# arkCyber/whisper-rust

Measured on AMD Instinct MI355X. Metric: real-time factor (audio-sec/wall-sec), greedy, 30 s synthetic chunks, higher is better.
Workload: dtype f16 operands / f32 accumulate; 1 GPU; ggml-small-shaped synthetic F16 model, greedy best_of=1 temperature_inc=0, 1 x 30 s 16 kHz f32 chunk per GPU, PCM resident in HBM; flash_attn=False, parallelism=chunk-dp1

## Files before the change

### whisper-rust_amd/csrc/wa_mega.h

```cpp
#pragma once
#include "wa_kernels.h"

struct wa_mega_layer {
    const float * ln1_w, * ln1_b; const wa_f16 * qkv_w; const float * qkv_b, * qkv_s;
    const wa_f16 * out_w;  const float * out_b;
    const float * ln2_w, * ln2_b; const wa_f16 * cq_w;  const float * cq_b;
    const wa_f16 * co_w;   const float * co_b;
    const float * ln3_w, * ln3_b; const wa_f16 * fc1_w; const float * fc1_b;
    const wa_f16 * fc2_w;  const float * fc2_b;
    const float * qkv_d, * out_d, * cq_d, * co_d, * fc1_d, * fc2_d;
};

struct wa_mega_args {
    const wa_mega_layer * layers; int n_layer, d, n_head, n_vocab; float eps;
    double rn_d;
    const wa_f16 * te; const float * pe; const float * lnf_w, * lnf_b; const wa_f16 * gelu;
    const float * te_d; int quant;
    wa_f16 * kv_k, * kv_v; unsigned long long kv_layer_stride;
    const wa_f16 * cross_k, * cross_v; unsigned long long cross_layer_stride;
    int cross_tpad, T;
    unsigned long long * granules; int edge_stride;
    unsigned long long * cross_gr;
    float * logits;
    unsigned * status;
// ... 30 lines not shown
        if (b < nG) { role = 0; idx = b; } else if (b < nG + H) { role = 1; idx = b - nG; } else { role = 2; idx = b - nG - H; }
        return;
    }
    if (b >= top) {
        const int t = b - top, r = t & 7, k = t >> 3, q = k >> 2, w = k & 3, h = r + 8 * q;
        if (h < H) { role = 2; idx = 4 * h + w; return; }
        const int f = (r - R) + (8 - R) * w;
        if (f < H) { role = 1; idx = f; } else { role = 0; idx = (top - s_low) + (f - H); }
        return;
    }
    if (b >= top - s_low) { role = 1; idx = F + (b - (top - s_low)); } else { role = 0; idx = b; }
}

bool   wa_launch_decode_mega(hipStream_t s, const wa_mega_args & a, int n_wg);
size_t wa_mega_lds_bytes();
```

### whisper-rust_amd/csrc/wa_mega.hip

```cpp
#include "wa_device.h"
#include "wa_mega.h"

typedef unsigned long long u64;
#define GAS __attribute__((address_space(1)))
typedef GAS u64 gu64;
typedef GAS unsigned gu32;
typedef const GAS wa_f16 * gch;
typedef const GAS float * gcf;
typedef _Float16 half4v __attribute__((ext_vector_type(4)));
typedef unsigned u32x2 __attribute__((ext_vector_type(2)));
typedef unsigned u32x4 __attribute__((ext_vector_type(4)));

typedef const __attribute__((address_space(4))) wa_mega_args * mg_kargs;
__device__ __forceinline__ mg_kargs mg_uniform(mg_kargs p) {
    const unsigned long long v = (unsigned long long) p;
    const unsigned lo = __builtin_amdgcn_readfirstlane((unsigned) v), hi = __builtin_amdgcn_readfirstlane((unsigned) (v >> 32));
    return (mg_kargs) (((unsigned long long) hi << 32) | lo);
}

#define MG_THREADS 512
#define MG_NW (MG_THREADS / 64)
#define MG_NP3 4
#define MG_SPIN_LIMIT 20000u
#ifndef MG_DEFER
// ... 75 lines not shown
        if ((spins & 127u) == 127u) {
            const unsigned st = __builtin_amdgcn_readfirstlane(__hip_atomic_load(c.status, __ATOMIC_RELAXED, __HIP_MEMORY_SCOPE_AGENT));
            if (st != 0u) { c.dead = true; return spins; }
            if (spins >= MG_SPIN_LIMIT) {
                if (lane == 0) __hip_atomic_store(c.status, code, __ATOMIC_RELAXED, __HIP_MEMORY_SCOPE_AGENT);
                c.dead = true;
                return spins;
            }
        }
        __builtin_amdgcn_s_sleep(1);
    }
}

#define MG_WGTRACE_LAYER 4
#define MG_NQ 6
#define MG_EX_P1 (MG_DEFER ? 0x06u : 0x20u)
#define MG_EX_P4 (MG_DEFER ? 0x06u : 0x08u)
#define MG_EX_P7 (BIGP ? 0x18u : MG_DEFER && !QB ? 0x10u : 0x08u)
#define MG_EX_AO 0x06u
#define MG_EX_AO2 0x10u
#define MG_EX_HF (MG_DEFER ? 0x08u : 0x06u)
#define MG_EX_HFQ 0x18u
#define MG_EX_FINAL 0x20u
__device__ __forceinline__ int mg_slot(int wave, unsigned ex) {
    if ((ex >> wave) & 1u) return -1;
    const int sl = __builtin_popcount(~ex & ((1u << wave) - 1u) & 0xffu);
    return sl < MG_NQ ? sl : -1;
}
__device__ __forceinline__ int mg_seg(int n) { return ((n + MG_NQ - 1) / MG_NQ + 31) & ~31; }
__device__ __forceinline__ int mg_ln_seg(int d) { return mg_seg(d); }
template <int NP3>
__device__ __forceinline__ void mg_ln_params(float (&gw)[NP3], float (&gb)[NP3], const float * lw, const float * lb, int d, int q, int lane) {
    const int seg = mg_ln_seg(d), i0 = q * seg, i1 = min(d, i0 + seg);
#pragma unroll
    for (int k = 0; k < NP3; ++k) {
        const int i = i0 + lane + 64 * k;
// ... 92 lines not shown
            else if (i < i1) xin[i] = f2h(y);
        }
        if (tslot >= 0) mg_trace(A, lane == 0, tslot + 2, mg_now());
    }
    mg_barrier();
}

template <int NPL>
__device__ __forceinline__ void mg_gather_h2(mg_ctl & c, gu64 * edge, int i0, int i1, int lane, unsigned * dst32, unsigned code, mg_kargs A = nullptr,
                                             int tslot = -1) {
    unsigned v[NPL];
    const unsigned sp = mg_sweep<NPL>(edge, [&](int k) { const int i = i0 + lane + 64 * k; return i < i1 ? i : -1; }, c, lane, v, code);
    if (tslot >= 0) { mg_trace(A, lane == 0, tslot, mg_now()); mg_trace(A, lane == 0, tslot + 1, sp); }
#pragma unroll
    for (int k = 0; k < NPL; ++k) { const int i = i0 + lane + 64 * k; if (i < i1) dst32[i] = v[k]; }
}

template <int NPL>
__device__ __forceinline__ void mg_gather_q8(mg_ctl & c, gu64 * edge, int i0, int i1, int lane, wa_f16 * xin, int nb, unsigned code, mg_kargs A = nullptr,
                                             int tslot = -1) {
    unsigned v[NPL];
    const unsigned sp = mg_sweep<NPL>(edge, [&](int k) { const int i = i0 + lane + 64 * k; return i < i1 ? i : -1; }, c, lane, v, code);
    if (tslot >= 0) { mg_trace(A, lane == 0, tslot, mg_now()); mg_trace(A, lane == 0, tslot + 1, sp); }
    const int ln = mq_fresh(lane);
    unsigned * q32 = (unsigned *) mq_xq(xin) + ((ln & 31) >> 2) * mq_ld(nb) + (i0 >> 5) + (ln >> 5);
    float * dsc = mq_xd(xin) + (i0 >> 5) + (ln >> 5);
#pragma unroll
    for (int k = 0; k < NPL; ++k) mq_put(__uint_as_float(v[k]), i0 + ln + 64 * k < i1, q32 + 2 * k, dsc + 2 * k, ln);
}

// ... 410 lines not shown
                                sl = __uint_as_float(rb[lane * 8 + 4]); ml = s2.v; }
            mg_best_wave(t2); mg_best_wave(s2);
            float sg = ml > -INFINITY ? sl * __expf(ml - s2.v) : 0.0f;
            sg = wave_sum(sg);
            if (lane == 0) {
                GAS unsigned * ro = (GAS unsigned *) A->rec_out + (size_t) wg * 8;
                ro[0] = __float_as_uint(t2.v); ro[1] = (unsigned) t2.i; ro[2] = __float_as_uint(s2.v); ro[3] = (unsigned) s2.i; ro[4] = __float_as_uint(sg);
            }
        }
    }
    mg_trace(A, blockIdx.x == 0 && wave == 0 && lane == 0, (A->n_layer * 8) * 8 + 3, mg_now());
    if (A->dbg) { mg_trace(A, blockIdx.x == 0 && wave == 0 && lane == 0, 3022, (unsigned) clock64()); mg_trace(A, blockIdx.x == 0 && wave == 0 && lane == 0, 3023, mg_now()); }
    if (blockIdx.x == 0 && wave == 0 && lane == 0) ((GAS unsigned *) A->logits)[A->n_vocab + 2] = c.seq;
}

template <int NP3, int NS, bool Q = false>
__device__ __forceinline__ void mg_role_gemv(mg_kargs A_, int idx_) {
    extern __shared__ __attribute__((aligned(16))) unsigned char smem[];
    const mg_kargs A = mg_uniform(A_);
    int lane = threadIdx.x & 63;
#define MG_FRESH() do { lane = mq_fresh(lane); } while (0)
    const int wave = __builtin_amdgcn_readfirstlane(threadIdx.x >> 6);
    const int wg = __builtin_amdgcn_readfirstlane(idx_), nG = (int) gridDim.x - 5 * A->n_head;
    mg_ctl c; c.status = (gu32 *) A->status; c.seq = A->seq; c.dead = false;
    mg_chaos_start(c.seq);
    mg_trace(A, wg == 0 && wave == 0 && (threadIdx.x & 63) == 0, (A->n_layer * 8) * 8 + 6, mg_now());
    if (A->dbg) { mg_trace(A, wg == 0 && wave == 0 && (threadIdx.x & 63) == 0, 3020, (unsigned) clock64()); mg_trace(A, wg == 0 && wave == 0 && (threadIdx.x & 63) == 0, 3021, mg_now()); }
    unsigned pf[96];
    bool have_pf = false;
    constexpr bool BIG = NP3 == MG_NP3;
    constexpr bool QB = Q && !BIG && MG_DEFER;
    constexpr bool BIGP = BIG && MG_DEFER;
    float    * fc1x   = (float *) (smem + WA_MEGA_MAX_D * 4 + 7 * WA_MEGA_MAX_D);
    unsigned * fc1cnt = (unsigned *) (smem + WA_MEGA_MAX_D * 4 + 7 * WA_MEGA_MAX_D + 128);

    float  * xf  = (float *) smem;
    wa_f16 * xin = (wa_f16 *) (smem + WA_MEGA_MAX_D * 4);
    wa_f16 * xinB = (wa_f16 *) (smem + MG_XINB_OFF);
    const int d = A->d, L = A->n_layer, d4 = 4 * d;
    const int r_qkv = mg_rpw(3 * d, nG), r_d = mg_rpw(d, nG), r_ff = mg_rpw(d4, nG);
    const int row_qkv = wg * r_qkv, row_d = wg * r_d, row_ff = wg * r_ff;
    const int g_qkv = (r_qkv + 7) >> 3, g_ff = (r_ff + 7) >> 3, g_d8 = (r_d + 7) >> 3, g_d16 = (r_d + 3) >> 2;
    const __attribute__((address_space(4))) wa_mega_layer * Ly = (const __attribute__((address_space(4))) wa_mega_layer *) A->layers;
    const unsigned seq = c.seq;
    const int kv_head = A->kv_head;

    double * lnred = (double *) (smem + MG_LNRED_OFF);
    wa_f16 * gelu_l = (wa_f16 *) (smem + MG_GELU_OFF);
    float gw[NP3], gb[NP3];
    int * pk = (int *) (smem + MG_PICK_OFF);
    mg_ln_params<NP3>(gw, gb, Ly[0].ln1_w, Ly[0].ln1_b, d, mg_slot(wave, MG_EX_P1), lane);
    if (wave == 0) mg_pick(A, lane, pk);
    if (QB && wave == 0 && lane == 0) *fc1cnt = 0u;
    mg_task t; t.valid = false; t.row = 0; t.wrow = nullptr; t.bias = 0.f; t.scale = 1.f;
    if (wave == 1 || wave == 2) t = mg_mk8<Q, NS>(pf, Ly[0].qkv_w, Ly[0].qkv_d, Ly[0].qkv_b, Ly[0].qkv_s, 3 * d, d, row_qkv, r_qkv, wave - 1, lane);
    else if (wave == 3)         t = mg_mk8<Q, NS>(pf, Ly[0].out_w, Ly[0].out_d, Ly[0].out_b, nullptr, d, d, row_d, r_d, 0, lane);
    else if (wave == 4)         t = mg_mk8<Q, NS>(pf, Ly[0].cq_w, Ly[0].cq_d, Ly[0].cq_b, nullptr, d, d, row_d, r_d, 0, lane);
    else if (wave == 5)         t = mg_mk16<Q, 4 * NS>(pf, Ly[0].fc2_w, Ly[0].fc2_d, Ly[0].fc2_b, d, d4, row_d, r_d, 0, lane);
    else if (wave >= 6 && !(BIGP && L > 0)) mg_prefetch_logits<NS, Q>(A, pf, have_pf, lane, wave);
    mg_barrier();
    mg_trace(A, wg == 0 && wave == 0 && lane == 0, (A->n_layer * 8) * 8 + 7, mg_now());
    if (wave >= 3 && wave <= 5) {
        const GAS u32x4 * src = (const GAS u32x4 *) A->gelu;
        for (int j = wave - 3; j < 128; j += 3)
            __builtin_amdgcn_global_load_lds((const GAS void *) (src + j * 64 + lane), (__attribute__((address_space(3))) void *) (smem + MG_GELU_OFF + (size_t) j * 1024), 16, 0, 0);
    }

    for (int l = 0; l < L; ++l) {
        const __attribute__((address_space(4))) wa_mega_layer & Y = Ly[l];
        auto big_next = [&](int w) {
            if (w - 2 < g_d16) t = mg_mk16<Q, 4 * NS>(pf, Y.fc2_w, Y.fc2_d, Y.fc2_b, d, d4, row_d, r_d, w - 2, lane);
            else if (l + 1 >= L) mg_prefetch_logits<NS, Q>(A, pf, have_pf, lane, w);
            else t = w == 3 ? mg_mk8<Q, NS>(pf, Ly[l + 1].out_w, Ly[l + 1].out_d, Ly[l + 1].out_b, nullptr, d, d, row_d, r_d, 0, lane)
                            : mg_mk8<Q, NS>(pf, Ly[l + 1].cq_w, Ly[l + 1].cq_d, Ly[l + 1].cq_b, nullptr, d, d, row_d, r_d, 0, lane);
        };
        MG_FRESH();
        mg_ln3<NP3, Q>(A, c, l == 0 ? nullptr : mg_edge(A, l - 1, E_X3), gw, gb, mg_slot(wave, MG_EX_P1), lane, xf, xinB, lnred, 100u + l, wg == 0 && wave == 0 ? (l * 8 + 0) * 8 : -1, pk[0]);
        MG_FRESH();
        mg_ln_params<NP3>(gw, gb, Y.ln2_w, Y.ln2_b, d, mg_slot(wave, MG_EX_P4), lane);
        if (MG_DEFER && l > 0 && wave == 5) t = mg_mk16<Q, 4 * NS>(pf, Y.fc2_w, Y.fc2_d, Y.fc2_b, d, d4, row_d, r_d, 0, lane);
        if (wave == 1 || wave == 2 || (BIG && (wave == 3 || wave == 4))) {
            const bool own = !BIG || wave <= 2;
            bool assisted = false;
            gu64 * eq = mg_edge(A, l, E_QKV);
            for (int grp = wave - 1; grp < g_qkv; grp += BIG ? 4 : 2) {
                if (grp >= 2) { t = mg_mk8<Q, NS>(pf, Y.qkv_w, Y.qkv_d, Y.qkv_b, Y.qkv_s, 3 * d, d, row_qkv, r_qkv, grp, lane); assisted = true; }
                MG_CHAOS_AT(1u);
                float v = mg_do8<Q, NS>(pf, t, d >> 5, xinB, lane);
                v = v + t.bias;
                v = v * t.scale;
                const unsigned pk = mg_pub_h2(eq, seq, t.valid, t.row, (unsigned) f2h(v), lane);
                if (t.valid && (lane & 15) == 0 && t.row >= d) {
                    GAS wa_f16 * cell = (t.row < 2 * d ? (GAS wa_f16 *) A->kv_k + (t.row - d) : (GAS wa_f16 *) A->kv_v + (t.row - 2 * d)) +
                                        (size_t) l * A->kv_layer_stride + (size_t) kv_head * d;
                    *(GAS unsigned *) cell = pk;
                }
            }
            mg_trace(A, wg == 0 && wave == 1 && lane == 0, (l * 8 + 0) * 8 + 3, mg_now());
            if (own && !MG_DEFER) t = mg_mk8<Q, NS>(pf, Y.fc1_w, Y.fc1_d, Y.fc1_b, nullptr, d4, d, row_ff, r_ff, wave - 1, lane);
            else if (assisted) t = wave == 3 ? mg_mk8<Q, NS>(pf, Y.out_w, Y.out_d, Y.out_b, nullptr, d, d, row_d, r_d, 0, lane)
                                             : mg_mk8<Q, NS>(pf, Y.cq_w, Y.cq_d, Y.cq_b, nullptr, d, d, row_d, r_d, 0, lane);
        }
        MG_FRESH();
        {
            const int qs = mg_slot(wave, MG_EX_AO), sg = mg_seg(Q ? 9 * (d >> 5) : d >> 1), j0 = qs * sg, j1 = min(Q ? 9 * (d >> 5) : d >> 1, j0 + sg);
            if constexpr (Q) { if (qs >= 0) mg_gather_qb<1>(c, mg_edge(A, l, E_AO), j0, j1, lane, xin, d >> 5, 200u + l, A, wg == 0 && wave == 0 ? (l * 8 + 1) * 8 : -1); }
            else if (qs >= 0) mg_gather_h2<2>(c, mg_edge(A, l, E_AO), j0, j1, lane, (unsigned *) xin, 200u + l, A, wg == 0 && wave == 0 ? (l * 8 + 1) * 8 : -1);
        }
        mg_barrier();
        MG_FRESH();
        if (MG_DEFER && (wave == 1 || wave == 2)) t = mg_mk8<Q, NS>(pf, Y.fc1_w, Y.fc1_d, Y.fc1_b, nullptr, d4, d, QB ? 32 * wg : row_ff, QB ? 32 : r_ff, wave - 1, lane);
        if (wave == 3 || (BIG && wave == 5)) {
            const bool own = !BIG || wave == 3;
            bool assisted = false;
            gu64 * ex = mg_edge(A, l, E_X1);
            for (int grp = own ? 0 : 1; grp < g_d8; grp += BIG ? 2 : 1) {
                if (grp >= 1) { t = mg_mk8<Q, NS>(pf, Y.out_w, Y.out_d, Y.out_b, nullptr, d, d, row_d, r_d, grp, lane); assisted = true; }
                MG_CHAOS_AT(2u);
                float v = mg_do8<Q, NS>(pf, t, d >> 5, xin, lane);
                v = v + t.bias;
                if (t.valid && (lane & 7) == 0) gr_store(ex + t.row, seq, __float_as_uint(v + xf[t.row]));
            }
            mg_trace(A, wg == 0 && own && lane == 0, (l * 8 + 1) * 8 + 3, mg_now());
            if (A->dbg && l == MG_WGTRACE_LAYER) mg_trace(A, own && lane == 0, 1024 + wg * 8 + 3, mg_now());
            if (own && !MG_DEFER) t = mg_mk8<Q, NS>(pf, Y.co_w, Y.co_d, Y.co_b, nullptr, d, d, row_d, r_d, 0, lane);
            else if (assisted) t = mg_mk16<Q, 4 * NS>(pf, Y.fc2_w, Y.fc2_d, Y.fc2_b, d, d4, row_d, r_d, 0, lane);
        }
        MG_FRESH();
        mg_ln3<NP3, Q>(A, c, mg_edge(A, l, E_X1), gw, gb, mg_slot(wave, MG_EX_P4), lane, xf, xinB, lnred, 300u + l,
                       wave == 0 ? (wg == 0 ? (l * 8 + 2) * 8 : (A->dbg && l == MG_WGTRACE_LAYER ? 1024 + wg * 8 : -1)) : -1);
        MG_FRESH();
        if (MG_DEFER && wave == 3) t = mg_mk8<Q, NS>(pf, Y.co_w, Y.co_d, Y.co_b, nullptr, d, d, row_d, r_d, 0, lane);
        if (BIGP && wave >= 6 && wave - 2 < g_ff) t = mg_mk8<Q, NS>(pf, Y.fc1_w, Y.fc1_d, Y.fc1_b, nullptr, d4, d, row_ff, r_ff, wave - 2, lane);
        mg_ln_params<NP3>(gw, gb, Y.ln3_w, Y.ln3_b, d, mg_slot(wave, MG_EX_P7), lane);
        if (wave == 4 || (BIG && wave == 3)) {
            const bool own = !BIG || wave == 4;
            bool assisted = false;
            gu64 * eq = mg_edge(A, l, E_QC);
            for (int grp = own ? 0 : 1; grp < g_d8; grp += BIG ? 2 : 1) {
                if (grp >= 1) { t = mg_mk8<Q, NS>(pf, Y.cq_w, Y.cq_d, Y.cq_b, nullptr, d, d, row_d, r_d, grp, lane); assisted = true; }
                MG_CHAOS_AT(3u);
                float v = mg_do8<Q, NS>(pf, t, d >> 5, xinB, lane);
                v = v + t.bias;
                mg_pub_h2(eq, seq, t.valid, t.row, (unsigned) f2h(v), lane);
            }
            mg_trace(A, wg == 0 && own && lane == 0, (l * 8 + 2) * 8 + 3, mg_now());
            if (A->dbg && l == MG_WGTRACE_LAYER) mg_trace(A, own && lane == 0, 1024 + wg * 8 + 6, mg_now());
            if (QB) t = mg_mk8<Q, NS>(pf, Y.fc1_w, Y.fc1_d, Y.fc1_b, nullptr, d4, d, 32 * wg, 32, 3, lane);
            else if (own && !MG_DEFER) {
                if (l + 1 < L) t = mg_mk8<Q, NS>(pf, Ly[l + 1].cq_w, Ly[l + 1].cq_d, Ly[l + 1].cq_b, nullptr, d, d, row_d, r_d, 0, lane);
                else mg_prefetch_logits<NS, Q>(A, pf, have_pf, lane, wave);
            } else if (assisted) t = mg_mk8<Q, NS>(pf, Y.co_w, Y.co_d, Y.co_b, nullptr, d, d, row_d, r_d, 0, lane);
        }
        MG_FRESH();
        {
            const int qs = mg_slot(wave, MG_EX_AO2), sg = mg_seg(Q ? 9 * (d >> 5) : d >> 1), j0 = qs * sg, j1 = min(Q ? 9 * (d >> 5) : d >> 1, j0 + sg);
            if constexpr (Q) { if (qs >= 0) mg_gather_qb<1>(c, mg_edge(A, l, E_AO2), j0, j1, lane, xin, d >> 5, 400u + l, A, wg == 0 && wave == 0 ? (l * 8 + 3) * 8 : -1); }
            else if (qs >= 0) mg_gather_h2<2>(c, mg_edge(A, l, E_AO2), j0, j1, lane, (unsigned *) xin, 400u + l, A, wg == 0 && wave == 0 ? (l * 8 + 3) * 8 : -1);
        }
        mg_barrier();
        MG_FRESH();
        if (MG_DEFER && !QB && !BIGP && wave == 4) {
            if (l + 1 < L) t = mg_mk8<Q, NS>(pf, Ly[l + 1].cq_w, Ly[l + 1].cq_d, Ly[l + 1].cq_b, nullptr, d, d, row_d, r_d, 0, lane);
            else mg_prefetch_logits<NS, Q>(A, pf, have_pf, lane, wave);
        }
        if (wave == 3 || (BIG && wave == 4)) {
            const bool own = !BIG || wave == 3;
            bool assisted = false;
            gu64 * ex = mg_edge(A, l, E_X2);
            for (int grp = own ? 0 : 1; grp < g_d8; grp += BIG ? 2 : 1) {
                if (grp >= 1) { t = mg_mk8<Q, NS>(pf, Y.co_w, Y.co_d, Y.co_b, nullptr, d, d, row_d, r_d, grp, lane); assisted = true; }
                MG_CHAOS_AT(4u);
                float v = mg_do8<Q, NS>(pf, t, d >> 5, xin, lane);
                v = v + t.bias;
                if (t.valid && (lane & 7) == 0) gr_store(ex + t.row, seq, __float_as_uint(v + xf[t.row]));
            }
            mg_trace(A, wg == 0 && own && lane == 0, (l * 8 + 3) * 8 + 3, mg_now());
            if (A->dbg && l == MG_WGTRACE_LAYER) mg_trace(A, own && lane == 0, 4096 + wg * 8 + 3, mg_now());
            if (QB) t = mg_mk8<Q, NS>(pf, Y.fc1_w, Y.fc1_d, Y.fc1_b, nullptr, d4, d, 32 * wg, 32, 2, lane);
            else if (BIGP) {
                if (wave - 1 < g_ff) t = mg_mk8<Q, NS>(pf, Y.fc1_w, Y.fc1_d, Y.fc1_b, nullptr, d4, d, row_ff, r_ff, wave - 1, lane);
                else big_next(wave);
            } else if (own && !MG_DEFER) {
                if (l + 1 < L) t = mg_mk8<Q, NS>(pf, Ly[l + 1].out_w, Ly[l + 1].out_d, Ly[l + 1].out_b, nullptr, d, d, row_d, r_d, 0, lane);
                else mg_prefetch_logits<NS, Q>(A, pf, have_pf, lane, wave);
            } else if (assisted) {
                if (l + 1 < L) t = mg_mk8<Q, NS>(pf, Ly[l + 1].cq_w, Ly[l + 1].cq_d, Ly[l + 1].cq_b, nullptr, d, d, row_d, r_d, 0, lane);
                else mg_prefetch_logits<NS, Q>(A, pf, have_pf, lane, wave);
            }
        }
        MG_FRESH();
        if (l == 0 && wave >= 3 && wave <= 5) asm volatile("s_waitcnt vmcnt(0)" ::: "memory");
        mg_ln3<NP3, Q>(A, c, mg_edge(A, l, E_X2), gw, gb, mg_slot(wave, MG_EX_P7), lane, xf, xinB, lnred, 500u + l,
                       wave == 0 ? (wg == 0 ? (l * 8 + 4) * 8 : (A->dbg && l == MG_WGTRACE_LAYER ? 4096 + wg * 8 : -1)) : -1);
        MG_FRESH();
        if (MG_DEFER && !QB && !BIGP && wave == 3) {
            if (l + 1 < L) t = mg_mk8<Q, NS>(pf, Ly[l + 1].out_w, Ly[l + 1].out_d, Ly[l + 1].out_b, nullptr, d, d, row_d, r_d, 0, lane);
            else mg_prefetch_logits<NS, Q>(A, pf, have_pf, lane, wave);
        }
        if (l + 1 < L) mg_ln_params<NP3>(gw, gb, Ly[l + 1].ln1_w, Ly[l + 1].ln1_b, d, mg_slot(wave, MG_EX_P1), lane);
        else           mg_ln_params<NP3>(gw, gb, A->lnf_w, A->lnf_b, d, mg_slot(wave, MG_EX_FINAL), lane);
        if (QB) {
            if (wave >= 1 && wave <= 4) {
                MG_CHAOS_AT(5u);
                float v = mg_do8<Q, NS>(pf, t, d >> 5, xinB, lane);
                v = v + t.bias;
                float gl = v;
                if (v <= -10.0f) gl = 0.0f; else if (v < 10.0f) gl = h2f(gelu_l[t.valid ? f2h(v) : 0]);
                if ((lane & 7) == 0) fc1x[8 * (wave - 1) + (lane >> 3)] = gl;
                MG_CHAOS_AT(51u);
                unsigned arrived = 0;
// ... 48 lines not shown
            for (int grp = wave - 1; grp < g_ff; grp += BIG ? 4 : 2) {
                if (grp >= 2) { t = mg_mk8<Q, NS>(pf, Y.fc1_w, Y.fc1_d, Y.fc1_b, nullptr, d4, d, row_ff, r_ff, grp, lane); assisted = true; }
                MG_CHAOS_AT(7u);
                float v = mg_do8<Q, NS>(pf, t, d >> 5, xinB, lane);
                v = v + t.bias;
                float gl = v;
                if (v <= -10.0f) gl = 0.0f; else if (v < 10.0f) gl = h2f(gelu_l[t.valid ? f2h(v) : 0]);
                if constexpr (Q) { if (t.valid && (lane & 7) == 0) gr_store(eh + t.row, seq, __float_as_uint(gl)); }
                else mg_pub_h2(eh, seq, t.valid, t.row, (unsigned) f2h(gl), lane);
            }
            mg_trace(A, wg == 0 && wave == 1 && lane == 0, (l * 8 + 4) * 8 + 3, mg_now());
            if (A->dbg && l == MG_WGTRACE_LAYER) mg_trace(A, wave == 1 && lane == 0, 4096 + wg * 8 + 6, mg_now());
            if (own && !MG_DEFER) {
                if (l + 1 < L) t = mg_mk8<Q, NS>(pf, Ly[l + 1].qkv_w, Ly[l + 1].qkv_d, Ly[l + 1].qkv_b, Ly[l + 1].qkv_s, 3 * d, d, row_qkv, r_qkv, wave - 1, lane);
                else mg_prefetch_logits<NS, Q>(A, pf, have_pf, lane, wave);
            } else if (assisted) {
                if (l + 1 >= L) mg_prefetch_logits<NS, Q>(A, pf, have_pf, lane, wave);
                else t = wave == 3 ? mg_mk8<Q, NS>(pf, Ly[l + 1].out_w, Ly[l + 1].out_d, Ly[l + 1].out_b, nullptr, d, d, row_d, r_d, 0, lane)
                                   : mg_mk8<Q, NS>(pf, Ly[l + 1].cq_w, Ly[l + 1].cq_d, Ly[l + 1].cq_b, nullptr, d, d, row_d, r_d, 0, lane);
            }
        }
        MG_FRESH();
        {
            const int ng = QB ? 9 * (d4 >> 5) : Q ? d4 : 2 * d;
            const int qs = mg_slot(wave, QB || BIGP ? MG_EX_HFQ : MG_EX_HF), sg = mg_seg(ng), i0 = qs * sg, i1 = min(ng, i0 + sg);
            if constexpr (QB) { if (qs >= 0) mg_gather_qb<3>(c, mg_edge(A, l, E_HF), i0, i1, lane, xin, d4 >> 5, 600u + l, A, wg == 0 && wave == 0 ? (l * 8 + 5) * 8 : -1); }
            else if constexpr (Q) { if (qs >= 0) mg_gather_q8<(NP3 == MG_NP3 ? 14 : 8)>(c, mg_edge(A, l, E_HF), i0, i1, lane, xin, d4 >> 5, 600u + l, A, wg == 0 && wave == 0 ? (l * 8 + 5) * 8 : -1); }
            else if (qs >= 0) mg_gather_h2<7>(c, mg_edge(A, l, E_HF), i0, i1, lane, (unsigned *) xin, 600u + l, A, wg == 0 && wave == 0 ? (l * 8 + 5) * 8 : -1);
        }
        mg_barrier();
        MG_FRESH();
        mg_trace(A, wg == 0 && wave == 5 && lane == 0, (l * 8 + 5) * 8 + 4, mg_now());
        if (MG_DEFER && (wave == 1 || wave == 2)) {
            if (l + 1 < L) t = mg_mk8<Q, NS>(pf, Ly[l + 1].qkv_w, Ly[l + 1].qkv_d, Ly[l + 1].qkv_b, Ly[l + 1].qkv_s, 3 * d, d, row_qkv, r_qkv, wave - 1, lane);
            else mg_prefetch_logits<NS, Q>(A, pf, have_pf, lane, wave);
        }
        if (wave == 5 || (BIG && (wave == 3 || wave == 4))) {
            const bool own = !BIG || wave == 5;
            bool assisted = false;
            gu64 * ex = mg_edge(A, l, E_X3);
            for (int grp = own ? 0 : wave - 2; grp < g_d16; grp += BIG ? 3 : 1) {
                if (grp >= (BIGP ? 3 : 1)) t = mg_mk16<Q, 4 * NS>(pf, Y.fc2_w, Y.fc2_d, Y.fc2_b, d, d4, row_d, r_d, grp, lane);
                if (grp >= 1) assisted = true;
                MG_CHAOS_AT(8u);
                float v = mg_do16<Q, 4 * NS>(pf, t, d4 >> 5, xin, lane);
                v = v + t.bias;
                if (t.valid && (lane & 15) == MG_RES16(Q)) gr_store(ex + t.row, seq, __float_as_uint(v + xf[t.row]));
            }
// ... 208 lines not shown
    }
    unsigned pf[96];
    bool have_pf = false;
    float gw[MG_NP3], gb[MG_NP3];
    if (wave >= 1) mg_prefetch_logits<0, Q>(A, pf, have_pf, lane, wave);
    mg_ln_params<MG_NP3>(gw, gb, A->lnf_w, A->lnf_b, A->d, mg_slot(wave, MG_EX_FINAL), lane);
    mg_final<MG_NP3, 0, Q>(A, c, smem, pf, have_pf, gw, gb, lane, wave);
}

#define MG_CSTEPS 48
#define MG_CGR 2048
#define MG_CGR_MAX 0
#define MG_CGR_SUM 8
#define MG_CGR_XCC 16
#define MG_CGR_PART 64

template <bool Q = false>
__device__ __forceinline__ void mg_role_cross(mg_kargs A_, int idx_) {
    extern __shared__ __attribute__((aligned(16))) unsigned char smem[];
    const mg_kargs A = mg_uniform(A_);
    const int tid = threadIdx.x, lane = tid & 63;
    const int wave = __builtin_amdgcn_readfirstlane(tid >> 6);
    const int H = A->n_head;
    const int ci = __builtin_amdgcn_readfirstlane(idx_);
    const int h = ci >> 2, w = ci & 3;
    mg_ctl c; c.status = (gu32 *) A->status; c.seq = A->seq; c.dead = false;
    mg_chaos_start(c.seq);
    const unsigned seq = c.seq;

    float  * part  = (float *) smem;
    wa_f16 * vleft = (wa_f16 *) (smem + 8192);
    float  * sc    = (float *) (smem + 8192 + 4096);
    wa_f16 * p16   = (wa_f16 *) (smem + 8192 + 4096 + 1536);
    wa_f16 * pleft = (wa_f16 *) (smem + 8192 + 4096 + 1536 + 768);
    wa_f16 * qs    = (wa_f16 *) (smem + 8192 + 4096 + 1536 + 768 + 64);
    double * redd  = (double *) (smem + 8192 + 4096 + 1536 + 768 + 64 + 128);
    float  * red   = (float *) (smem + 8192 + 4096 + 1536 + 768 + 64 + 128 + 64);
    float  * bc    = red + 8;

    const int T = A->T, tpad = A->cross_tpad, L = A->n_layer;
    const float kq_scale = A->kq_scale;
    const int a = tid & 3, ks = tid >> 2;
    const int np = T & ~31, nsteps = np >> 5, nl = T - np, n8 = T & ~7, ng = n8 >> 3;
    if (wave == 0) mg_pick(A, lane, (int *) (smem + MG_PICK_OFF));
    if (wave == 0) {
        const unsigned xcc = (unsigned) __builtin_amdgcn_s_getreg(20 | (3 << 11)) & 0xfu;
        gu64 * X0 = (gu64 *) A->cross_gr + (size_t) h * MG_CGR + MG_CGR_XCC;
        if (lane == 0) gr_store(X0 + w, seq, xcc);
        unsigned v[1];
        mg_sweep<1>(X0, [&](int) { return lane < 4 ? lane : -1; }, c, lane, v, 2900u);
        const bool same = lane >= 4 || v[0] == xcc;
        if (lane == 0) bc[2] = __builtin_amdgcn_ballot_w64(same) == ~0ull && !c.dead ? 1.0f : 0.0f;
    }
    mg_barrier();
    const bool local = bc[2] != 0.0f;
    for (int l = 0; l < L; ++l) {
        gu64 * X = (gu64 *) A->cross_gr + ((size_t) l * H + h) * MG_CGR;
        const gch kp = (gch) A->cross_k + (size_t) l * A->cross_layer_stride + (size_t) h * tpad * 64;
        const gch vp = (gch) A->cross_v + (size_t) l * A->cross_layer_stride + (size_t) h * tpad * 64;
        u32x4 ka[3], kb[3];
        unsigned short vv[MG_CSTEPS];
#pragma unroll
        for (int p = 0; p < 3; ++p) {
            const int o = p * 128 + ks, cc = 32 * (o >> 3) + 8 * w + (o & 7);
            if (cc < T) { ka[p] = *(const GAS u32x4 *) (kp + (size_t) cc * 64 + 8 * a); kb[p] = *(const GAS u32x4 *) (kp + (size_t) cc * 64 + 32 + 8 * a); }
        }
#pragma unroll
        for (int s = 0; s < MG_CSTEPS; ++s) if (s < nsteps) vv[s] = *(const GAS unsigned short *) (vp + (size_t) (32 * s + 8 * w + wave) * 64 + lane);
        if (w == 0 && tid < 256) {
            const int row = tid >> 3;
            if (row < nl) *(u32x4 *) (vleft + (size_t) tid * 8) = *(const GAS u32x4 *) (vp + (size_t) (np + row) * 64 + (tid & 7) * 8);
        }
        if (wave == 0) {
            unsigned v[1];
            mg_trace(A, ci == 0 && lane == 0, (l * 8 + 7) * 8 + 2, mg_now());
            const unsigned sp = mg_sweep<1>(mg_edge(A, l, E_QC), [&](int) { return lane < 32 ? h * 32 + lane : -1; }, c, lane, v, 2000u + l);
            mg_trace(A, ci == 0 && lane == 0, (l * 8 + 7) * 8 + 0, mg_now()); mg_trace(A, ci == 0 && lane == 0, (l * 8 + 7) * 8 + 1, sp);
            if (A->dbg && l == MG_WGTRACE_LAYER && w == 0) mg_trace(A, lane == 0, 3200 + h, mg_now());
            if (lane < 32) ((unsigned *) qs)[lane] = v[0];
        }
        mg_barrier();
#define MG_CX(k) do { if (A->dbg && l == MG_WGTRACE_LAYER) mg_trace(A, ci == 0 && tid == 0, 3010 + (k), mg_now()); } while (0)
        MG_CX(0);
        MG_CHAOS_ID(2000 + ci, 31u, seq);
        float lmax = -INFINITY;
        {
            float qa[8], qb[8];
#pragma unroll
// ... 100 lines not shown
            mg_attn_finish<Q>(part, vleft, pleft - np, np, nl, mg_edge(A, l, E_AO2), h, seq, tid, (double *) (smem + 16384), (double *) (smem + 24576), A,
                              A->dbg && ci == 0 && l == MG_WGTRACE_LAYER ? 3000 : -1);
            mg_trace(A, ci == 0 && tid == 0, (l * 8 + 7) * 8 + 3, mg_now());
            if (A->dbg && l == MG_WGTRACE_LAYER) mg_trace(A, tid == 0, 3100 + h, mg_now());
        }
        mg_barrier();
    }
    unsigned pf[96];
    bool have_pf = false;
    float gw[MG_NP3], gb[MG_NP3];
    if (wave >= 1) mg_prefetch_logits<0, Q>(A, pf, have_pf, lane, wave);
    mg_ln_params<MG_NP3>(gw, gb, A->lnf_w, A->lnf_b, A->d, mg_slot(wave, MG_EX_FINAL), lane);
    mg_final<MG_NP3, 0, Q>(A, c, smem, pf, have_pf, gw, gb, lane, wave);
}

__global__ __launch_bounds__(MG_THREADS) void k_decode_mega(const wa_mega_args A) {
    int role, idx;
    mg_role_of((int) gridDim.x, A.n_head, (int) blockIdx.x, role, idx);
    const mg_kargs Ap = (mg_kargs) __builtin_amdgcn_kernarg_segment_ptr();
    if (role == 0) {
        if (A.d == 768) mg_role_gemv<2, 24>(Ap, idx); else if (A.d < 768) mg_role_gemv<2, 0>(Ap, idx);
        else mg_role_gemv<MG_NP3, 0>(Ap, idx);
    }
    else if (role == 1) mg_role_self(Ap, idx);
    else                mg_role_cross(Ap, idx);
}

__global__ __launch_bounds__(MG_THREADS) void k_decode_mega_q(const wa_mega_args A) {
    int role, idx;
    mg_role_of((int) gridDim.x, A.n_head, (int) blockIdx.x, role, idx);
    const mg_kargs Ap = (mg_kargs) __builtin_amdgcn_kernarg_segment_ptr();
    if (role == 0) {
        if (A.d == 768) mg_role_gemv<2, 24, true>(Ap, idx); else if (A.d < 768) mg_role_gemv<2, 0, true>(Ap, idx);
        else if (A.d == 1280) mg_role_gemv<MG_NP3, 40, true>(Ap, idx); else mg_role_gemv<MG_NP3, 0, true>(Ap, idx);
    }
    else if (role == 1) mg_role_self<true>(Ap, idx);
    else                mg_role_cross<true>(Ap, idx);
}

size_t wa_mega_lds_bytes() {
    const size_t s_self  = (size_t) WA_MEGA_MAX_KV * 64 * 2 * 2 + MG_ATT_SMEM(WA_MEGA_MAX_KV);
    const size_t s_cross = 32768;
    const size_t s_gemv  = MG_PICK_OFF;
    size_t m = s_self > s_cross ? s_self : s_cross;
    m = m > s_gemv ? m : s_gemv;
    if (m > MG_PICK_OFF || (MG_PICK_OFF & 255) != 0) abort();
    return MG_PICK_OFF + MG_PICK_BYTES;
}

bool wa_launch_decode_mega(hipStream_t s, const wa_mega_args & a, int n_wg) {
    static bool attr_set[64] = {};
    const size_t lds = wa_mega_lds_bytes();
    int dev = 0;
    (void) hipGetDevice(&dev);
    if (!attr_set[dev & 63]) {
        if (hipFuncSetAttribute((const void *) k_decode_mega, hipFuncAttributeMaxDynamicSharedMemorySize, (int) lds) != hipSuccess ||
            hipFuncSetAttribute((const void *) k_decode_mega_q, hipFuncAttributeMaxDynamicSharedMemorySize, (int) lds) != hipSuccess) return false;
        attr_set[dev & 63] = true;
    }
    if (a.quant) hipLaunchKernelGGL(k_decode_mega_q, dim3(n_wg), dim3(MG_THREADS), lds, s, a);
    else         hipLaunchKernelGGL(k_decode_mega, dim3(n_wg), dim3(MG_THREADS), lds, s, a);
    return hipGetLastError() == hipSuccess;
}
```

Baseline: 337.9 x real-time.

## Fuse cross-attention query projection and LN2 into cross-attention workgroups for d=768

Adds a CQ variant of the decode megakernel for the F16 d=768 case. In it, each cross-attention workgroup computes LN2 and its own head's slice of the cross-query projection locally, instead of waiting on a grid-wide QC edge published by GEMV workgroups. The GEMV role drops its cq work and re-schedules waves for qkv, out and co prefetch. This removes one inter-workgroup sync stage per layer, at the cost of each cross workgroup redundantly gathering X1 and doing LN plus extra weight reads. It also needs a separate translation unit (MG_CQ_TU) to be compiled and linked.

```diff
diff --git a/whisper-rust_amd/csrc/wa_mega.h b/whisper-rust_amd/csrc/wa_mega.h
--- a/whisper-rust_amd/csrc/wa_mega.h
+++ b/whisper-rust_amd/csrc/wa_mega.h
@@ -68,3 +68,4 @@
 
 bool   wa_launch_decode_mega(hipStream_t s, const wa_mega_args & a, int n_wg);
 size_t wa_mega_lds_bytes();
+bool   wa_launch_decode_mega_cq(hipStream_t s, const wa_mega_args & a, int n_wg, size_t lds);
diff --git a/whisper-rust_amd/csrc/wa_mega.hip b/whisper-rust_amd/csrc/wa_mega.hip
--- a/whisper-rust_amd/csrc/wa_mega.hip
+++ b/whisper-rust_amd/csrc/wa_mega.hip
@@ -113,12 +113,13 @@
 
 #define MG_WGTRACE_LAYER 4
 #define MG_NQ 6
-#define MG_EX_P1 (MG_DEFER ? 0x06u : 0x20u)
+#define MG_EX_P1 (CQ ? 0x20u : MG_DEFER ? 0x06u : 0x20u)
 #define MG_EX_P4 (MG_DEFER ? 0x06u : 0x08u)
 #define MG_EX_P7 (BIGP ? 0x18u : MG_DEFER && !QB ? 0x10u : 0x08u)
-#define MG_EX_AO 0x06u
-#define MG_EX_AO2 0x10u
-#define MG_EX_HF (MG_DEFER ? 0x08u : 0x06u)
+#define MG_EX_AO (CQ ? 0xc0u : 0x06u)
+#define MG_EX_AO2 (CQ ? 0xc0u : 0x10u)
+#define MG_EX_HF (CQ ? 0x06u : MG_DEFER ? 0x08u : 0x06u)
+#define MG_EX_X1 0x06u
 #define MG_EX_HFQ 0x18u
 #define MG_EX_FINAL 0x20u
 __device__ __forceinline__ int mg_slot(int wave, unsigned ex) {
@@ -241,6 +242,15 @@
     if (tslot >= 0) { mg_trace(A, lane == 0, tslot, mg_now()); mg_trace(A, lane == 0, tslot + 1, sp); }
 #pragma unroll
     for (int k = 0; k < NPL; ++k) { const int i = i0 + lane + 64 * k; if (i < i1) dst32[i] = v[k]; }
+}
+
+template <int NPL>
+__device__ __forceinline__ void mg_gather_f32(mg_ctl & c, gu64 * edge, int i0, int i1, int lane, float * dst, unsigned code, mg_kargs A = nullptr, int tslot = -1) {
+    unsigned v[NPL];
+    const unsigned sp = mg_sweep<NPL>(edge, [&](int k) { const int i = i0 + lane + 64 * k; return i < i1 ? i : -1; }, c, lane, v, code);
+    if (tslot >= 0) { mg_trace(A, lane == 0, tslot, mg_now()); mg_trace(A, lane == 0, tslot + 1, sp); }
+#pragma unroll
+    for (int k = 0; k < NPL; ++k) { const int i = i0 + lane + 64 * k; if (i < i1) dst[i] = __uint_as_float(v[k]); }
 }
 
 template <int NPL>
@@ -681,7 +691,7 @@
     if (blockIdx.x == 0 && wave == 0 && lane == 0) ((GAS unsigned *) A->logits)[A->n_vocab + 2] = c.seq;
 }
 
-template <int NP3, int NS, bool Q = false>
+template <int NP3, int NS, bool Q = false, bool CQ = false>
 __device__ __forceinline__ void mg_role_gemv(mg_kargs A_, int idx_) {
     extern __shared__ __attribute__((aligned(16))) unsigned char smem[];
     const mg_kargs A = mg_uniform(A_);
@@ -698,6 +708,7 @@
     constexpr bool BIG = NP3 == MG_NP3;
     constexpr bool QB = Q && !BIG && MG_DEFER;
     constexpr bool BIGP = BIG && MG_DEFER;
+    static_assert(!CQ || (!Q && !BIG && MG_DEFER), "the CQ form is the F16 small-width schedule");
     float    * fc1x   = (float *) (smem + WA_MEGA_MAX_D * 4 + 7 * WA_MEGA_MAX_D);
     unsigned * fc1cnt = (unsigned *) (smem + WA_MEGA_MAX_D * 4 + 7 * WA_MEGA_MAX_D + 128);
 
@@ -720,11 +731,12 @@
     if (wave == 0) mg_pick(A, lane, pk);
     if (QB && wave == 0 && lane == 0) *fc1cnt = 0u;
     mg_task t; t.valid = false; t.row = 0; t.wrow = nullptr; t.bias = 0.f; t.scale = 1.f;
-    if (wave == 1 || wave == 2) t = mg_mk8<Q, NS>(pf, Ly[0].qkv_w, Ly[0].qkv_d, Ly[0].qkv_b, Ly[0].qkv_s, 3 * d, d, row_qkv, r_qkv, wave - 1, lane);
+    if (CQ && L > 0 && wave >= 6) t = mg_mk8<Q, NS>(pf, Ly[0].qkv_w, Ly[0].qkv_d, Ly[0].qkv_b, Ly[0].qkv_s, 3 * d, d, row_qkv, r_qkv, wave - 6, lane);
+    else if ((wave == 1 || wave == 2) && !CQ) t = mg_mk8<Q, NS>(pf, Ly[0].qkv_w, Ly[0].qkv_d, Ly[0].qkv_b, Ly[0].qkv_s, 3 * d, d, row_qkv, r_qkv, wave - 1, lane);
     else if (wave == 3)         t = mg_mk8<Q, NS>(pf, Ly[0].out_w, Ly[0].out_d, Ly[0].out_b, nullptr, d, d, row_d, r_d, 0, lane);
-    else if (wave == 4)         t = mg_mk8<Q, NS>(pf, Ly[0].cq_w, Ly[0].cq_d, Ly[0].cq_b, nullptr, d, d, row_d, r_d, 0, lane);
+    else if (wave == 4 && !CQ)  t = mg_mk8<Q, NS>(pf, Ly[0].cq_w, Ly[0].cq_d, Ly[0].cq_b, nullptr, d, d, row_d, r_d, 0, lane);
     else if (wave == 5)         t = mg_mk16<Q, 4 * NS>(pf, Ly[0].fc2_w, Ly[0].fc2_d, Ly[0].fc2_b, d, d4, row_d, r_d, 0, lane);
-    else if (wave >= 6 && !(BIGP && L > 0)) mg_prefetch_logits<NS, Q>(A, pf, have_pf, lane, wave);
+    else if (wave >= 6 && !((BIGP || CQ) && L > 0)) mg_prefetch_logits<NS, Q>(A, pf, have_pf, lane, wave);
     mg_barrier();
     mg_trace(A, wg == 0 && wave == 0 && lane == 0, (A->n_layer * 8) * 8 + 7, mg_now());
     if (wave >= 3 && wave <= 5) {
@@ -744,13 +756,13 @@
         MG_FRESH();
         mg_ln3<NP3, Q>(A, c, l == 0 ? nullptr : mg_edge(A, l - 1, E_X3), gw, gb, mg_slot(wave, MG_EX_P1), lane, xf, xinB, lnred, 100u + l, wg == 0 && wave == 0 ? (l * 8 + 0) * 8 : -1, pk[0]);
         MG_FRESH();
-        mg_ln_params<NP3>(gw, gb, Y.ln2_w, Y.ln2_b, d, mg_slot(wave, MG_EX_P4), lane);
+        if (!CQ) mg_ln_params<NP3>(gw, gb, Y.ln2_w, Y.ln2_b, d, mg_slot(wave, MG_EX_P4), lane);
         if (MG_DEFER && l > 0 && wave == 5) t = mg_mk16<Q, 4 * NS>(pf, Y.fc2_w, Y.fc2_d, Y.fc2_b, d, d4, row_d, r_d, 0, lane);
-        if (wave == 1 || wave == 2 || (BIG && (wave == 3 || wave == 4))) {
+        if (CQ ? wave >= 6 : wave == 1 || wave == 2 || (BIG && (wave == 3 || wave == 4))) {
             const bool own = !BIG || wave <= 2;
             bool assisted = false;
             gu64 * eq = mg_edge(A, l, E_QKV);
-            for (int grp = wave - 1; grp < g_qkv; grp += BIG ? 4 : 2) {
+            for (int grp = CQ ? wave - 6 : wave - 1; grp < g_qkv; grp += BIG ? 4 : 2) {
                 if (grp >= 2) { t = mg_mk8<Q, NS>(pf, Y.qkv_w, Y.qkv_d, Y.qkv_b, Y.qkv_s, 3 * d, d, row_qkv, r_qkv, grp, lane); assisted = true; }
                 MG_CHAOS_AT(1u);
                 float v = mg_do8<Q, NS>(pf, t, d >> 5, xinB, lane);
@@ -763,7 +775,7 @@
                     *(GAS unsigned *) cell = pk;
                 }
             }
-            mg_trace(A, wg == 0 && wave == 1 && lane == 0, (l * 8 + 0) * 8 + 3, mg_now());
+            mg_trace(A, wg == 0 && wave == (CQ ? 6 : 1) && lane == 0, (l * 8 + 0) * 8 + 3, mg_now());
             if (own && !MG_DEFER) t = mg_mk8<Q, NS>(pf, Y.fc1_w, Y.fc1_d, Y.fc1_b, nullptr, d4, d, row_ff, r_ff, wave - 1, lane);
             else if (assisted) t = wave == 3 ? mg_mk8<Q, NS>(pf, Y.out_w, Y.out_d, Y.out_b, nullptr, d, d, row_d, r_d, 0, lane)
                                              : mg_mk8<Q, NS>(pf, Y.cq_w, Y.cq_d, Y.cq_b, nullptr, d, d, row_d, r_d, 0, lane);
@@ -794,13 +806,26 @@
             else if (assisted) t = mg_mk16<Q, 4 * NS>(pf, Y.fc2_w, Y.fc2_d, Y.fc2_b, d, d4, row_d, r_d, 0, lane);
         }
         MG_FRESH();
+        if constexpr (CQ) {
+            const int qs = mg_slot(wave, MG_EX_X1), sg = mg_seg(d), i0 = qs * sg, i1 = min(d, i0 + sg);
+            if (qs >= 0) mg_gather_f32<NP3>(c, mg_edge(A, l, E_X1), i0, i1, lane, xf, 300u + l, A,
+                                            wave == 0 ? (wg == 0 ? (l * 8 + 2) * 8 : (A->dbg && l == MG_WGTRACE_LAYER ? 1024 + wg * 8 : -1)) : -1);
+            mg_barrier();
+            MG_FRESH();
+            if (wave == 4) t = mg_mk8<Q, NS>(pf, Y.co_w, Y.co_d, Y.co_b, nullptr, d, d, row_d, r_d, 0, lane);
+            else if (wave == 3 || wave >= 6) {
+                if (l + 1 >= L) mg_prefetch_logits<NS, Q>(A, pf, have_pf, lane, wave);
+                else if (wave == 3) t = mg_mk8<Q, NS>(pf, Ly[l + 1].out_w, Ly[l + 1].out_d, Ly[l + 1].out_b, nullptr, d, d, row_d, r_d, 0, lane);
+                else t = mg_mk8<Q, NS>(pf, Ly[l + 1].qkv_w, Ly[l + 1].qkv_d, Ly[l + 1].qkv_b, Ly[l + 1].qkv_s, 3 * d, d, row_qkv, r_qkv, wave - 6, lane);
+            }
+        } else
         mg_ln3<NP3, Q>(A, c, mg_edge(A, l, E_X1), gw, gb, mg_slot(wave, MG_EX_P4), lane, xf, xinB, lnred, 300u + l,
                        wave == 0 ? (wg == 0 ? (l * 8 + 2) * 8 : (A->dbg && l == MG_WGTRACE_LAYER ? 1024 + wg * 8 : -1)) : -1);
         MG_FRESH();
-        if (MG_DEFER && wave == 3) t = mg_mk8<Q, NS>(pf, Y.co_w, Y.co_d, Y.co_b, nullptr, d, d, row_d, r_d, 0, lane);
+        if (MG_DEFER && !CQ && wave == 3) t = mg_mk8<Q, NS>(pf, Y.co_w, Y.co_d, Y.co_b, nullptr, d, d, row_d, r_d, 0, lane);
         if (BIGP && wave >= 6 && wave - 2 < g_ff) t = mg_mk8<Q, NS>(pf, Y.fc1_w, Y.fc1_d, Y.fc1_b, nullptr, d4, d, row_ff, r_ff, wave - 2, lane);
         mg_ln_params<NP3>(gw, gb, Y.ln3_w, Y.ln3_b, d, mg_slot(wave, MG_EX_P7), lane);
-        if (wave == 4 || (BIG && wave == 3)) {
+        if (!CQ && (wave == 4 || (BIG && wave == 3))) {
             const bool own = !BIG || wave == 4;
             bool assisted = false;
             gu64 * eq = mg_edge(A, l, E_QC);
@@ -827,11 +852,11 @@
         }
         mg_barrier();
         MG_FRESH();
-        if (MG_DEFER && !QB && !BIGP && wave == 4) {
+        if (MG_DEFER && !QB && !BIGP && !CQ && wave == 4) {
             if (l + 1 < L) t = mg_mk8<Q, NS>(pf, Ly[l + 1].cq_w, Ly[l + 1].cq_d, Ly[l + 1].cq_b, nullptr, d, d, row_d, r_d, 0, lane);
             else mg_prefetch_logits<NS, Q>(A, pf, have_pf, lane, wave);
         }
-        if (wave == 3 || (BIG && wave == 4)) {
+        if (wave == (CQ ? 4 : 3) || (BIG && wave == 4)) {
             const bool own = !BIG || wave == 3;
             bool assisted = false;
             gu64 * ex = mg_edge(A, l, E_X2);
@@ -845,6 +870,7 @@
             mg_trace(A, wg == 0 && own && lane == 0, (l * 8 + 3) * 8 + 3, mg_now());
             if (A->dbg && l == MG_WGTRACE_LAYER) mg_trace(A, own && lane == 0, 4096 + wg * 8 + 3, mg_now());
             if (QB) t = mg_mk8<Q, NS>(pf, Y.fc1_w, Y.fc1_d, Y.fc1_b, nullptr, d4, d, 32 * wg, 32, 2, lane);
+            else if (CQ) { if (l + 1 >= L) mg_prefetch_logits<NS, Q>(A, pf, have_pf, lane, wave); }
             else if (BIGP) {
                 if (wave - 1 < g_ff) t = mg_mk8<Q, NS>(pf, Y.fc1_w, Y.fc1_d, Y.fc1_b, nullptr, d4, d, row_ff, r_ff, wave - 1, lane);
                 else big_next(wave);
@@ -861,7 +887,7 @@
         mg_ln3<NP3, Q>(A, c, mg_edge(A, l, E_X2), gw, gb, mg_slot(wave, MG_EX_P7), lane, xf, xinB, lnred, 500u + l,
                        wave == 0 ? (wg == 0 ? (l * 8 + 4) * 8 : (A->dbg && l == MG_WGTRACE_LAYER ? 4096 + wg * 8 : -1)) : -1);
         MG_FRESH();
-        if (MG_DEFER && !QB && !BIGP && wave == 3) {
+        if (MG_DEFER && !QB && !BIGP && !CQ && wave == 3) {
             if (l + 1 < L) t = mg_mk8<Q, NS>(pf, Ly[l + 1].out_w, Ly[l + 1].out_d, Ly[l + 1].out_b, nullptr, d, d, row_d, r_d, 0, lane);
             else mg_prefetch_logits<NS, Q>(A, pf, have_pf, lane, wave);
         }
@@ -940,6 +966,8 @@
             if (own && !MG_DEFER) {
                 if (l + 1 < L) t = mg_mk8<Q, NS>(pf, Ly[l + 1].qkv_w, Ly[l + 1].qkv_d, Ly[l + 1].qkv_b, Ly[l + 1].qkv_s, 3 * d, d, row_qkv, r_qkv, wave - 1, lane);
                 else mg_prefetch_logits<NS, Q>(A, pf, have_pf, lane, wave);
+            } else if (CQ) {
+                if (l + 1 >= L) mg_prefetch_logits<NS, Q>(A, pf, have_pf, lane, wave);
             } else if (assisted) {
                 if (l + 1 >= L) mg_prefetch_logits<NS, Q>(A, pf, have_pf, lane, wave);
                 else t = wave == 3 ? mg_mk8<Q, NS>(pf, Ly[l + 1].out_w, Ly[l + 1].out_d, Ly[l + 1].out_b, nullptr, d, d, row_d, r_d, 0, lane)
@@ -957,7 +985,7 @@
         mg_barrier();
         MG_FRESH();
         mg_trace(A, wg == 0 && wave == 5 && lane == 0, (l * 8 + 5) * 8 + 4, mg_now());
-        if (MG_DEFER && (wave == 1 || wave == 2)) {
+        if (MG_DEFER && !CQ && (wave == 1 || wave == 2)) {
             if (l + 1 < L) t = mg_mk8<Q, NS>(pf, Ly[l + 1].qkv_w, Ly[l + 1].qkv_d, Ly[l + 1].qkv_b, Ly[l + 1].qkv_s, 3 * d, d, row_qkv, r_qkv, wave - 1, lane);
             else mg_prefetch_logits<NS, Q>(A, pf, have_pf, lane, wave);
         }
@@ -1196,12 +1224,17 @@
 #define MG_CGR_SUM 8
 #define MG_CGR_XCC 16
 #define MG_CGR_PART 64
-
-template <bool Q = false>
+#define MG_CX_XF 32768
+#define MG_CX_XIN (MG_CX_XF + WA_MEGA_MAX_D * 4)
+#define MG_CX_LNRED (MG_CX_XIN + WA_MEGA_MAX_D * 2)
+#define MG_CX_END (MG_CX_LNRED + 256)
+#define MG_CX_TRACE 6144
+
+template <bool Q = false, int CQ = -1>
 __device__ __forceinline__ void mg_role_cross(mg_kargs A_, int idx_) {
     extern __shared__ __attribute__((aligned(16))) unsigned char smem[];
     const mg_kargs A = mg_uniform(A_);
-    const int tid = threadIdx.x, lane = tid & 63;
+    int tid = threadIdx.x, lane = tid & 63;
     const int wave = __builtin_amdgcn_readfirstlane(tid >> 6);
     const int H = A->n_head;
     const int ci = __builtin_amdgcn_readfirstlane(idx_);
@@ -1222,7 +1255,7 @@
 
     const int T = A->T, tpad = A->cross_tpad, L = A->n_layer;
     const float kq_scale = A->kq_scale;
-    const int a = tid & 3, ks = tid >> 2;
+    int a = tid & 3, ks = tid >> 2;
     const int np = T & ~31, nsteps = np >> 5, nl = T - np, n8 = T & ~7, ng = n8 >> 3;
     if (wave == 0) mg_pick(A, lane, (int *) (smem + MG_PICK_OFF));
     if (wave == 0) {
@@ -1236,7 +1269,16 @@
     }
     mg_barrier();
     const bool local = bc[2] != 0.0f;
+    const __attribute__((address_space(4))) wa_mega_layer * Ly = (const __attribute__((address_space(4))) wa_mega_layer *) A->layers;
+    float  * xf    = (float *) (smem + MG_CX_XF);
+    wa_f16 * xin   = (wa_f16 *) (smem + MG_CX_XIN);
+    double * lnred = (double *) (smem + MG_CX_LNRED);
+    const int d = A->d;
     for (int l = 0; l < L; ++l) {
+        if constexpr (CQ >= 0) {
+            unsigned z = threadIdx.x; asm volatile("" : "+v"(z));
+            tid = (int) z; lane = tid & 63; a = tid & 3; ks = tid >> 2;
+        }
         gu64 * X = (gu64 *) A->cross_gr + ((size_t) l * H + h) * MG_CGR;
         const gch kp = (gch) A->cross_k + (size_t) l * A->cross_layer_stride + (size_t) h * tpad * 64;
         const gch vp = (gch) A->cross_v + (size_t) l * A->cross_layer_stride + (size_t) h * tpad * 64;
@@ -1253,7 +1295,26 @@
             const int row = tid >> 3;
             if (row < nl) *(u32x4 *) (vleft + (size_t) tid * 8) = *(const GAS u32x4 *) (vp + (size_t) (np + row) * 64 + (tid & 7) * 8);
         }
-        if (wave == 0) {
+        if constexpr (CQ >= 0) {
+            unsigned pf[96];
+            float gw[2], gb[2];
+            const int row = 64 * h + 8 * wave + (lane >> 3);
+            const gch wrow = (gch) Ly[l].cq_w + (size_t) row * d + 4 * (lane & 7);
+            mg_pf8<CQ>(pf, wrow, true, d >> 5, 0);
+            const float bias = ((gcf) Ly[l].cq_b)[row];
+            mg_ln_params<2>(gw, gb, Ly[l].ln2_w, Ly[l].ln2_b, d, mg_slot(wave, 0u), lane);
+            mg_trace(A, ci == 0 && lane == 0 && wave == 0, (l * 8 + 7) * 8 + 2, mg_now());
+            mg_ln3<2>(A, c, mg_edge(A, l, E_X1), gw, gb, mg_slot(wave, 0u), lane, xf, xin, lnred, 2000u + l,
+                      ci == 0 && wave == 0 ? MG_CX_TRACE + l * 8 : -1);
+            MG_CHAOS_ID(2000 + ci, 30u, seq);
+            float v = mg_dot8<CQ>(pf, wrow, true, d >> 5, xin, lane & 7, true);
+            v = v + bias;
+            const unsigned hq = (unsigned) f2h(v);
+            if ((lane & 7) == 0) qs[8 * wave + (lane >> 3)] = (wa_f16) hq;
+            if (A->dbg && w == 0) mg_pub_h2(mg_edge(A, l, E_QC), seq, true, row, hq, lane);
+            mg_trace(A, ci == 0 && lane == 0 && wave == 0, (l * 8 + 7) * 8 + 0, mg_now());
+            if (A->dbg && l == MG_WGTRACE_LAYER && w == 0) mg_trace(A, tid == 0, 3200 + h, mg_now());
+        } else if (wave == 0) {
             unsigned v[1];
             mg_trace(A, ci == 0 && lane == 0, (l * 8 + 7) * 8 + 2, mg_now());
             const unsigned sp = mg_sweep<1>(mg_edge(A, l, E_QC), [&](int) { return lane < 32 ? h * 32 + lane : -1; }, c, lane, v, 2000u + l);
@@ -1384,6 +1445,7 @@
     mg_final<MG_NP3, 0, Q>(A, c, smem, pf, have_pf, gw, gb, lane, wave);
 }
 
+#ifndef MG_CQ_TU
 __global__ __launch_bounds__(MG_THREADS) void k_decode_mega(const wa_mega_args A) {
     int role, idx;
     mg_role_of((int) gridDim.x, A.n_head, (int) blockIdx.x, role, idx);
@@ -1396,6 +1458,7 @@
     else                mg_role_cross(Ap, idx);
 }
 
+
 __global__ __launch_bounds__(MG_THREADS) void k_decode_mega_q(const wa_mega_args A) {
     int role, idx;
     mg_role_of((int) gridDim.x, A.n_head, (int) blockIdx.x, role, idx);
@@ -1410,7 +1473,7 @@
 
 size_t wa_mega_lds_bytes() {
     const size_t s_self  = (size_t) WA_MEGA_MAX_KV * 64 * 2 * 2 + MG_ATT_SMEM(WA_MEGA_MAX_KV);
-    const size_t s_cross = 32768;
+    const size_t s_cross = MG_CX_END;
     const size_t s_gemv  = MG_PICK_OFF;
     size_t m = s_self > s_cross ? s_self : s_cross;
     m = m > s_gemv ? m : s_gemv;
@@ -1428,7 +1491,30 @@
             hipFuncSetAttribute((const void *) k_decode_mega_q, hipFuncAttributeMaxDynamicSharedMemorySize, (int) lds) != hipSuccess) return false;
         attr_set[dev & 63] = true;
     }
+    if (MG_DEFER && !a.quant && a.d == 768) return wa_launch_decode_mega_cq(s, a, n_wg, lds);
     if (a.quant) hipLaunchKernelGGL(k_decode_mega_q, dim3(n_wg), dim3(MG_THREADS), lds, s, a);
     else         hipLaunchKernelGGL(k_decode_mega, dim3(n_wg), dim3(MG_THREADS), lds, s, a);
     return hipGetLastError() == hipSuccess;
 }
+#else
+__global__ __launch_bounds__(MG_THREADS) void k_decode_mega_cq(const wa_mega_args A) {
+    int role, idx;
+    mg_role_of((int) gridDim.x, A.n_head, (int) blockIdx.x, role, idx);
+    const mg_kargs Ap = (mg_kargs) __builtin_amdgcn_kernarg_segment_ptr();
+    if (role == 0)      mg_role_gemv<2, 24, false, true>(Ap, idx);
+    else if (role == 1) mg_role_self(Ap, idx);
+    else                mg_role_cross<false, 24>(Ap, idx);
+}
+
+bool wa_launch_decode_mega_cq(hipStream_t s, const wa_mega_args & a, int n_wg, size_t lds) {
+    static bool attr_set[64] = {};
+    int dev = 0;
+    (void) hipGetDevice(&dev);
+    if (!attr_set[dev & 63]) {
+        if (hipFuncSetAttribute((const void *) k_decode_mega_cq, hipFuncAttributeMaxDynamicSharedMemorySize, (int) lds) != hipSuccess) return false;
+        attr_set[dev & 63] = true;
+    }
+    hipLaunchKernelGGL(k_decode_mega_cq, dim3(n_wg), dim3(MG_THREADS), lds, s, a);
+    return hipGetLastError() == hipSuccess;
+}
+#endif
```

New measurement: 350.6 x real-time (median of 6 runs). +3.8%, better.
